# mycophonic/saprobe-alac

Hardware: AMD Instinct MI355X
Metric: Msamples/s decoded (16-bit stereo, 4096-frame packets) (higher is better)
Workload: dtype int32; 1 GPU; 65536 packets/GPU x 16-bit 2-ch 4096-frame ALAC, music-like synthetic, device-resident in/out; packets_per_gpu=65536

## Files before the change

saprobe-alac_amd/csrc/alac_duo.h:

```cpp
#ifndef ALAC_DUO_H
#define ALAC_DUO_H

#include <type_traits>

#include "alac_regular.h"

namespace alac {

constexpr uint32_t DUO_CHUNK = 16;
constexpr int DUO_UN8_MAX = 12;
enum { ROLE_A = 0, ROLE_B = 1, ROLE_BOTH = 2, ROLE_C = 3 };

template <class W, class B, int NA, int OUT, int ROLE, bool F16, bool NARROW, bool EA, bool UN8W = false, bool EC = false, int WMODE = 0>
ALAC_DEV void duo_phase(W& wv, const DevCfg& cfg, const B& bits, RegLane<W>& s, uint32_t size, uint32_t ns,
                        uint32_t n_it, uint32_t hdr_pos, uint32_t den_shift, uint32_t chan_bits, int32_t mix_res,
                        uint32_t mix_sh, uint32_t na_rt, uint32_t shift_pos, uint32_t sb, uint32_t mode) {
    constexpr bool DO_A = ROLE == ROLE_A || ROLE == ROLE_BOTH, DO_B = ROLE == ROLE_B || ROLE == ROLE_BOTH;
    constexpr bool RAW = OUT == OUT_RAW;
    constexpr bool LAST = OUT == OUT_STEREO || OUT == OUT_MONO || RAW;
    constexpr bool CPE = OUT == OUT_STEREO;
    constexpr bool QND = W::kResMem || EC;
    constexpr bool GEN = NA == 0;
    constexpr int NR = GEN ? 1 : NA;
    constexpr bool WRAP = !(NA == 4 || NA == 5 || NA == 6 || NA == 8);
    constexpr uint32_t BIAS = 0x80000000u;
    static_assert(!(EA && EC), "one writer");
    constexpr bool DO_C = (ROLE == ROLE_C || ROLE == ROLE_BOTH) && EC;
    constexpr bool EMIT_A = (EA || EC) && LAST && !RAW;
    constexpr bool DO_EMIT = EMIT_A ? (EC ? DO_C : DO_A) : DO_B;
    constexpr uint32_t CH = EMIT_A ? DUO_CHUNK / 2u : DUO_CHUNK;
    const uint32_t na = GEN ? na_rt : (uint32_t)NA;
    uint32_t kb = cfg.kb;
    ALAC_OWN_REG(kb);
    const uint32_t wb = go_shl(1u, kb) - 1u;
    const uint32_t c31kb = 31u - kb;
    const uint32_t chan_shift = 32u - chan_bits;
    const int32_t den_half = den_shift ? (int32_t)(1u << (den_shift - 1u)) : 0;
    const uint32_t rnd_neg = (1u << den_shift) - 1u;

    int32_t coef[NR];
    uint32_t hb[NR + 1];
    if (DO_B) {
#pragma unroll
        for (int j = 0; j < NR; ++j)
            coef[j] = (!GEN || ((uint32_t)j < na && na != 31)) ? (int32_t)(int16_t)bits.get(hdr_pos + 16u + 16u * (uint32_t)j, 16) : 0;
#pragma unroll
        for (int j = 0; j <= NR; ++j) hb[j] = BIAS;
    }
    uint64_t pk_acc = 0;
    uint32_t pk_n = 0;
    const uint32_t bps = cfg.bps;
    const uint64_t pk_msk = bps == 4 ? 0xffffffffull : ((1ull << (8u * bps)) - 1ull);
    const bool merge_any = DO_EMIT && LAST && !F16 && !RAW && wv.any(sb != 0);
    const bool mode_any = DO_B && wv.any(mode != 0);
    int32_t dprev = 0;
    auto prepass = [&](uint32_t idx, int32_t del) -> int32_t {
        if (!mode_any) return del;
        const int32_t dd = idx == 0 ? del : sext_cs(del + dprev, chan_shift);
        dprev = mode != 0 ? dd : dprev;
        return mode != 0 ? dd : del;
    };
    constexpr bool MID_ONLY = !NARROW && WMODE == 1;
    const bool mid = !NARROW && (MID_ONLY || !wv.any(ns != 0u && chan_bits > 25u));
// ... 66 lines not shown
            const uint32_t pcm = ((uint32_t)l & 0xffffu) | ((uint32_t)r << 16);
            if (FP) wv.st_put(fp_base, jj, pcm, fp_inc);
            else wv.st_push_if(pcm, on);
            return;
        }
        if (cfg.bit_depth == 20) {
            l = (int32_t)((uint32_t)l << 4);
            r = (int32_t)((uint32_t)r << 4);
        }
        if (merge_any) {
            const uint32_t sh_l = sb ? (uint32_t)(sw >> (64u - sb)) : 0u;
            const uint32_t sh_r = (CPE && sb) ? (uint32_t)((sw << sb) >> (64u - sb)) : 0u;
            l = (int32_t)((uint32_t)l << sb) | (int32_t)sh_l;
            r = (int32_t)((uint32_t)r << sb) | (int32_t)sh_r;
        }
        {
            pk_acc |= ((uint64_t)(uint32_t)l & pk_msk) << (8u * pk_n);
            pk_n += on ? bps : 0u;
            bool em = pk_n >= 4u;
            wv.st_push_if((uint32_t)pk_acc, em);
            pk_acc = em ? pk_acc >> 32 : pk_acc;
            pk_n = em ? pk_n - 4u : pk_n;
            if (CPE) {
                pk_acc |= ((uint64_t)(uint32_t)r & pk_msk) << (8u * pk_n);
                pk_n += on ? bps : 0u;
                em = pk_n >= 4u;
                wv.st_push_if((uint32_t)pk_acc, em);
                pk_acc = em ? pk_acc >> 32 : pk_acc;
                pk_n = em ? pk_n - 4u : pk_n;
            }
            pk_acc &= pk_n ? ((1ull << (8u * pk_n)) - 1ull) : 0ull;
        }
    };
    auto put = [&](uint32_t buf, uint32_t j, uint32_t i, int32_t o, int32_t u, uint64_t sw, uint32_t jj, auto fp) {
#pragma unroll
        for (int t = NR; t >= 1; --t) hb[t] = hb[t - 1];
        hb[0] = (uint32_t)o ^ BIAS;
        if (!LAST) *wv.u_row(i) = o;
        else if (EMIT_A) wv.rq_write(buf, CH + j, o);
        else emit(i, o, u, sw, jj, fp);
    };
    constexpr bool PK3 = CPE && LAST && !F16 && !RAW && !EMIT_A;
    constexpr bool PK3C = CPE && LAST && !F16 && !RAW && EMIT_A && EC;
    const bool sb8 = (PK3 || PK3C) && !wv.any(ns != 0u && sb != 8u);
    const bool sb0 = (PK3 || PK3C) && !wv.any(ns != 0u && sb != 0u);
    const bool pk3 = (PK3 || PK3C) && bps == 3u && (sb8 || sb0);
    const uint32_t sh_byte = shift_pos >> 3, sh_bit = shift_pos & 7u;
    auto pk3_block = [&](uint32_t rowq, const int32_t (&vv4)[4], const int32_t (&uu4)[4], uint32_t g0, uint32_t g1, uint32_t g2) {
        const uint32_t w0 = (uint32_t)(((((uint64_t)g0) << 32) | g1) << sh_bit >> 32);
        const uint32_t w1 = (uint32_t)(((((uint64_t)g1) << 32) | g2) << sh_bit >> 32);
        uint32_t lq[4], rq[4];
#pragma unroll
        for (uint32_t j = 0; j < 4u; ++j) {
            const int32_t vv = vv4[j];
            const int32_t mv = NARROW ? ALAC_MUL24(mix_res, vv) : (int32_t)((uint32_t)mix_res * (uint32_t)vv);
            int32_t l = uu4[j] + (int32_t)((uint32_t)vv & nzm) - (mv >> mix_sh);
            int32_t r = (int32_t)((((uint32_t)(l - vv)) & nzm) | ((uint32_t)vv & ~nzm));
            if (sb8) {
                const uint32_t w = j < 2u ? w0 : w1;
                const uint32_t sl = (j & 1u) ? (w >> 8) & 0xffu : w >> 24;
                const uint32_t sr = (j & 1u) ? w & 0xffu : (w >> 16) & 0xffu;
                l = (int32_t)(((uint32_t)l << 8) | sl);
                r = (int32_t)(((uint32_t)r << 8) | sr);
            } else if (cfg.bit_depth == 20) {
                l = (int32_t)((uint32_t)l << 4);
                r = (int32_t)((uint32_t)r << 4);
            }
            lq[j] = (uint32_t)l;
            rq[j] = (uint32_t)r;
        }
        const uint32_t d0 = (lq[0] & 0xffffffu) | (rq[0] << 24);
// ... 47 lines not shown
            const uint32_t i = c * CH + j;
            u_n[j] = 0;
            sw_n[j] = 0;
            if (i < n_it) {
                if (CPE) u_n[j] = *wv.u_row(i);
                if (merge_any && !blocks) sw_n[j] = bits.window_raw(shift_pos + i * sstep_a);
            }
        }
        if (PK3C && blocks && sb8) {
#pragma unroll
            for (uint32_t q = 0; q < CH / 4u; ++q) bits.load12(sh_byte + 2u * (c * CH + 4u * q), g_n[q][0], g_n[q][1], g_n[q][2]);
        }
    };
    auto emit_chunk = [&](uint32_t c) {
        if (PK3C && whole_pk3(c)) {
#pragma unroll
            for (uint32_t q = 0; q < CH / 4u; ++q) {
                int32_t vv4[4], uu4[4];
#pragma unroll
                for (uint32_t j = 0; j < 4u; ++j) {
                    vv4[j] = sq_v[4u * q + j];
                    uu4[j] = u_v[4u * q + j];
                }
                pk3_block(c * CH + 4u * q, vv4, uu4, g_v[q][0], g_v[q][1], g_v[q][2]);
            }
            return;
        }
#pragma unroll
        for (uint32_t j = 0; j < CH; ++j) {
            const uint32_t i = c * CH + j;
            if (i < n_it) emit(i, sq_v[j], u_v[j], sw_v[j], 0u, fp_no{});
        }
        wv.st_step();
    };
    constexpr uint32_t UN = (NARROW && (((F16 || !LAST || RAW || EMIT_A) && NR <= DUO_UN8_MAX) || (UN8W && NR <= 8))) ? 8u : 4u;
    constexpr bool HBM_IN = LAST && !RAW && !EMIT_A;
    constexpr bool RMEM = W::kResMem && ROLE == ROLE_B;
    int32_t dpre[UN];
    uint32_t dpre_row = 0xffffffffu;
    int32_t upre[UN];
    uint64_t spre[UN];
    uint32_t pre_row = 0xffffffffu;
    constexpr uint32_t NSUB = UN / 4u;
    uint32_t gpre[NSUB][3] = {};
    auto prefetch_group = [&](uint32_t row0) {
        pre_row = row0;
#pragma unroll
        for (uint32_t j = 0; j < UN; ++j) {
            upre[j] = 0;
            spre[j] = 0;
            if (CPE) upre[j] = *wv.u_row(row0 + j);
            if (merge_any && !pk3) spre[j] = bits.window_raw(shift_pos + (row0 + j) * sstep_b);
        }
        if (PK3 && pk3 && sb8) {
#pragma unroll
            for (uint32_t q = 0; q < NSUB; ++q) bits.load12(sh_byte + 2u * (row0 + 4u * q), gpre[q][0], gpre[q][1], gpre[q][2]);
        }
    };
    auto predict_chunk = [&](uint32_t c) {
        const uint32_t buf = c & 1u;
        const bool simple = GEN && (na == 0 || na == 31);
        const uint32_t sstep = (CPE ? 2u : 1u) * sb;
        if (!simple && !mode_any && c * CH > na && (c + 1u) * CH <= n_it) {
            auto groups = [&](auto wrap, auto fp) {
                constexpr bool FP = decltype(fp)::value;
#pragma nounroll
// ... 13 lines not shown
                        uv[j] = HBM_IN ? upre[j] : 0;
                        sv[j] = HBM_IN ? spre[j] : 0ull;
                    }
                    uint32_t gq[NSUB][3];
#pragma unroll
                    for (uint32_t q = 0; q < NSUB; ++q) {
                        gq[q][0] = gpre[q][0];
                        gq[q][1] = gpre[q][1];
                        gq[q][2] = gpre[q][2];
                    }
                    if (HBM_IN && row0 + 2u * UN <= steady_end) prefetch_group(row0 + UN);
                    if (RMEM && row0 + 2u * UN <= steady_end) {
                        dpre_row = row0 + UN;
#pragma unroll
                        for (uint32_t j = 0; j < UN; ++j) dpre[j] = wv.rq_read(buf, g + UN + j);
                    }
                    if (PK3 && pk3) {
#pragma unroll
                        for (uint32_t q = 0; q < NSUB; ++q) {
                            int32_t vv4[4], uu4[4];
#pragma unroll
                            for (uint32_t j = 0; j < 4u; ++j) {
                                const int32_t vv = predict_q(dv[4u * q + j], wrap);
#pragma unroll
                                for (int t = NR; t >= 1; --t) hb[t] = hb[t - 1];
                                hb[0] = (uint32_t)vv ^ BIAS;
                                vv4[j] = vv;
                                uu4[j] = uv[4u * q + j];
                            }
                            pk3_block(row0 + 4u * q, vv4, uu4, gq[q][0], gq[q][1], gq[q][2]);
                        }
                        continue;
                    }
#pragma unroll
                    for (uint32_t j = 0; j < UN; ++j)
                        put(buf, g + j, c * CH + g + j, predict_q(dv[j], wrap), uv[j], sv[j], j, fp);
                    if (FP) wv.st_advance(fp_inc);
                    if (LAST && !EMIT_A) wv.st_step();
                }
            };
            auto run_groups = [&](auto wrap) {
                if (FP_OK) {
                    const uint32_t c_end = (c + 1u) * CH;
                    const bool ends_here = ns > c * CH && ns < c_end;
                    if (!wv.any(ends_here)) {
                        fp_inc = ns >= c_end ? UN : 0u;
                        groups(wrap, fp_yes{});
                        return;
                    }
                    groups(wrap, fp_no{});
                    if (ends_here) (void)wv.st_finish();
                    return;
                }
                groups(wrap, fp_no{});
            };
            if (WRAP) {
                constexpr uint32_t T = 32767u - CH;
                uint32_t far = 0;
#pragma unroll
                for (int j = 0; j < NR; ++j) far = umax(far, (uint32_t)coef[j] + T);
                if (!wv.any(far > 2u * T)) {
                    run_groups(wrap_no{});
                    return;
                }
            }
            run_groups(wrap_yes{});
            return;
        }
#pragma nounroll
        for (uint32_t j = 0; j < CH; ++j) {
            const uint32_t i = c * CH + j;
            if (i >= n_it) break;
            const int32_t qv = wv.rq_read(buf, j);
            const int32_t del = prepass(i, QND ? gol_unfold((uint32_t)qv) : qv);
            int32_t o;
            if (i == 0 || (GEN && na == 0)) o = del;
            else if (i <= na || (GEN && na == 31)) o = sext_cs(del + (int32_t)(hb[0] ^ BIAS), chan_shift);
            else o = predict(del, wrap_yes{});
            put(buf, j, i, o, (CPE && !EMIT_A) ? *wv.u_row(i) : 0,
                (!EMIT_A && merge_any) ? bits.window_raw(shift_pos + i * sstep) : 0ull, 0u, fp_no{});
            if (LAST && !EMIT_A) wv.st_step();
            if (FP_OK && i + 1u == ns) (void)wv.st_finish();
        }
    };

    const uint32_t nch = (n_it + CH - 1u) / CH;
    const uint32_t iters = nch + (EMIT_A ? 2u : 1u);
    for (uint32_t c = 0; c < iters; ++c) {
        if (DO_A) {
            if (EMIT_A && !EC && c >= 2u) fetch_chunk(c - 2u);
            if (c < nch) golomb_chunk(c);
        }
        if (DO_B) {
            if (c >= 1u && c <= nch) predict_chunk(c - 1u);
        }
        if (DO_A && EMIT_A && !EC) {
            if (c >= 2u) emit_chunk(c - 2u);
        }
        if (DO_C && EMIT_A) {
            if (c >= 2u) {
#pragma unroll
                for (uint32_t j = 0; j < CH; ++j) {
                    u_v[j] = u_n[j];
                    sw_v[j] = sw_n[j];
                }
#pragma unroll
                for (uint32_t q = 0; q < CH / 4u; ++q) {
                    g_v[q][0] = g_n[q][0];
                    g_v[q][1] = g_n[q][1];
                    g_v[q][2] = g_n[q][2];
                }
            }
            if (c >= 1u && c <= nch) fetch_mem_ahead(c - 1u);
            if (c >= 2u) {
                fetch_chunk(c - 2u);
                emit_chunk(c - 2u);
            }
        }
        wv.duo_sync();
    }
    if (DO_EMIT && LAST) wv.st_tail(pk_acc, pk_n);
    if (!LAST) wv.duo_sync_mem();
}

template <class W, class B, int T, int OUT, int LPP, int NAC = 0>
ALAC_DEV void duo_phase_lanes(W& wv, const B& bits, uint32_t q, uint32_t n_it, uint32_t hdr_pos, uint32_t den_shift,
                              uint32_t chan_bits, uint32_t na_rt) {
    static_assert(LPP == 2 || LPP == 4, "lanes per packet");
    static_assert(LPP == 2 ? NAC == 0 : (NAC >= 1 && (NAC + 3) / 4 == T), "four lanes: T = ceil(order / 4)");
    const uint32_t na = NAC != 0 ? (uint32_t)NAC : na_rt;
    constexpr bool LAST = OUT != OUT_UTILE;
    constexpr uint32_t CH = LAST ? DUO_CHUNK / 2u : DUO_CHUNK;
    constexpr uint32_t BIAS = 0x80000000u;
    const bool wraps = order_wraps16(na);
    const uint32_t chan_shift = 32u - chan_bits;
    const int32_t den_half = den_shift ? (int32_t)(1u << (den_shift - 1u)) : 0;
    const int32_t dh0 = q == 0u ? den_half : 0;
    const uint32_t rnd_neg = (1u << den_shift) - 1u;
    const uint32_t q0m = q == 0u ? 0xffffffffu : 0u;
    const uint32_t up1 = q < 3u ? 0xffffffffu : 0u, up2 = q < 2u ? 0xffffffffu : 0u, up3 = q < 1u ? 0xffffffffu : 0u;
    int32_t coef[T], wneg[T], m[T];
    uint32_t g[T + 1];
#pragma unroll
    for (int t = 0; t < T; ++t) {
        const uint32_t jt = q * (uint32_t)T + (uint32_t)t;
        const bool have = jt < na;
        coef[t] = have ? (int32_t)(int16_t)bits.get(hdr_pos + 16u + 16u * jt, 16) : 0;
        wneg[t] = have ? -(int32_t)(na - jt) : 0;
        m[t] = have ? 1 : 0;
        g[t] = BIAS;
    }
    g[T] = BIAS;
    int32_t prev = 0;
    constexpr int QTOP = NAC != 0 ? (NAC - 1) / T : 1, TTOP = NAC != 0 ? NAC - QTOP * T : T;
    const bool top_last = na == 2u * (uint32_t)T;

    auto step = [&](uint32_t i, uint32_t nd, auto plain_c, auto wrap_c) -> int32_t {
        constexpr bool PLAIN = decltype(plain_c)::value, WR = decltype(wrap_c)::value;
// ... 21 lines not shown
                s = ALAC_MAD24(qv[t], wneg[t], s);
            } else {
                acc = ALAC_MUL24(coef[t], e[t]) + acc;
                s = ALAC_MUL24((int32_t)qv[t], wneg[t]) + s;
            }
        }
        if (LPP == 2) rem += (int32_t)(wv.pair_hi((uint32_t)s) & q0m);
        else rem += (int32_t)((wv.template quad_up<1>((uint32_t)s) & up1) + (wv.template quad_up<2>((uint32_t)s) & up2) +
                              (wv.template quad_up<3>((uint32_t)s) & up3));
#pragma unroll
        for (int t = T - 1; t >= 0; --t) {
            const int32_t go = ALAC_MED3_0(rem, m[t]);
            const int32_t delta = (int32_t)ALAC_XAD(sg[t], sgnm, nsg);
            rem = ALAC_MAD24(qv[t], wneg[t], rem);
            int32_t cj = ALAC_MAD24(delta, go, coef[t]);
            if (WR) cj = (int32_t)(int16_t)cj;
            coef[t] = cj;
        }
        const int32_t at = LPP == 2 ? wv.pair_sum(acc) : wv.quad_sum(acc);
        int32_t o = ALAC_SEXT_BITS(del + (int32_t)(topb ^ BIAS) + (at >> den_shift), chan_bits);
        if (!PLAIN) {
            if (i == 0u) o = del;
            else if (i <= na) o = sext_cs(del + prev, chan_shift);
        }
        const uint32_t g0 = LPP == 2 ? wv.pair_from_below(g[T - 1], (uint32_t)o ^ BIAS, q0m) : wv.quad_from_below(g[T - 1], (uint32_t)o ^ BIAS, q0m);
#pragma unroll
        for (int t = T; t >= 1; --t) g[t] = g[t - 1];
        g[0] = g0;
        prev = o;
        return o;
    };
    using yes = std::integral_constant<bool, true>;
    using no = std::integral_constant<bool, false>;
    auto put = [&](uint32_t buf, uint32_t k, uint32_t i, int32_t o) {
        if (!LAST) *wv.u_row(i) = o;
        else wv.rq_write(buf, CH + k, o);
    };
    auto predict_chunk = [&](uint32_t cc) {
        const uint32_t i0 = cc * CH, buf = cc & 1u;
        const uint32_t nst = umin(CH, n_it - i0);
        if (i0 > na && nst == CH) {
            auto run = [&](auto wrap_c) {
                uint32_t dv[CH];
#pragma unroll
                for (uint32_t k = 0; k < CH; ++k) dv[k] = (uint32_t)wv.rq_read(buf, k);
#pragma unroll
                for (uint32_t k = 0; k < CH; ++k) put(buf, k, i0 + k, step(i0 + k, dv[k], yes{}, wrap_c));
            };
            if (wraps) {
                constexpr uint32_t TW = 32767u - CH;
                uint32_t far = 0;
#pragma unroll
                for (int t = 0; t < T; ++t) far = umax(far, (uint32_t)coef[t] + TW);
                if (wv.any(far > 2u * TW)) {
                    run(yes{});
                    return;
                }
            }
            run(no{});
            return;
        }
#pragma nounroll
        for (uint32_t k = 0; k < nst; ++k) {
            const uint32_t nd = (uint32_t)wv.rq_read(buf, k);
            const int32_t o = wraps ? step(i0 + k, nd, no{}, yes{}) : step(i0 + k, nd, no{}, no{});
            put(buf, k, i0 + k, o);
        }
    };
    const uint32_t nch = (n_it + CH - 1u) / CH;
    const uint32_t iters = nch + (LAST ? 2u : 1u);
    for (uint32_t c = 0; c < iters; ++c) {
        if (c >= 1u && c <= nch) predict_chunk(c - 1u);
        wv.duo_sync();
    }
    if (!LAST) wv.duo_sync_mem();
}

template <class W, int OUT, int LPP, class B>
ALAC_DEV void duo_phase_lanes_na(W& wv, uint32_t na, const B& bits, uint32_t q, uint32_t n_it, uint32_t hdr_pos, uint32_t den_shift,
                                 uint32_t chan_bits) {
    if constexpr (LPP == 4) {
#define ALAC_L4(N) \
    case N: duo_phase_lanes<W, B, (N + 3) / 4, OUT, 4, N>(wv, bits, q, n_it, hdr_pos, den_shift, chan_bits, na); break;
        switch (na) {
            ALAC_L4(3) ALAC_L4(4) ALAC_L4(5) ALAC_L4(6) ALAC_L4(7) ALAC_L4(8) ALAC_L4(9) ALAC_L4(10) ALAC_L4(11) ALAC_L4(12)
            ALAC_L4(13) ALAC_L4(14) ALAC_L4(15)
            default: duo_phase_lanes<W, B, 4, OUT, 4, 16>(wv, bits, q, n_it, hdr_pos, den_shift, chan_bits, na); break;
        }
#undef ALAC_L4
    } else {
        switch ((na + 1u) / 2u) {
            case 0:
            case 1:
            case 2: duo_phase_lanes<W, B, 2, OUT, 2>(wv, bits, q, n_it, hdr_pos, den_shift, chan_bits, na); break;
            case 3: duo_phase_lanes<W, B, 3, OUT, 2>(wv, bits, q, n_it, hdr_pos, den_shift, chan_bits, na); break;
            case 4: duo_phase_lanes<W, B, 4, OUT, 2>(wv, bits, q, n_it, hdr_pos, den_shift, chan_bits, na); break;
            case 5: duo_phase_lanes<W, B, 5, OUT, 2>(wv, bits, q, n_it, hdr_pos, den_shift, chan_bits, na); break;
            case 6: duo_phase_lanes<W, B, 6, OUT, 2>(wv, bits, q, n_it, hdr_pos, den_shift, chan_bits, na); break;
            case 7: duo_phase_lanes<W, B, 7, OUT, 2>(wv, bits, q, n_it, hdr_pos, den_shift, chan_bits, na); break;
            default: duo_phase_lanes<W, B, 8, OUT, 2>(wv, bits, q, n_it, hdr_pos, den_shift, chan_bits, na); break;
        }
    }
}

ALAC_DEV bool duo_lanes_key(uint32_t key, bool cpe, uint32_t lanes_min) {
    const uint32_t nu = (key >> 5) & 31u, nv = key & 31u;
    if ((key & KEY_WIDE) != 0u || nu < 3u || nu > 16u) return false;
    if (!cpe) return nu >= lanes_min;
    if (nv < 3u || nv > 16u) return false;
    return umax(nu, nv) >= lanes_min;
}

ALAC_DEV constexpr bool duo_emit_in_a(uint32_t na, bool cpe) { return !cpe && na >= 5u && na <= 16u; }

template <class W, int OUT, int ROLE, bool F16, bool NARROW = true, bool UN8W = false, bool EC = false, int WMODE = 0, class B>
ALAC_DEV void duo_phase_na(W& wv, uint32_t na, const DevCfg& cfg, const B& bits, RegLane<W>& s, uint32_t size,
                           uint32_t ns, uint32_t n_it, uint32_t hdr_pos, uint32_t den_shift, uint32_t chan_bits,
                           int32_t mix_res, uint32_t mix_sh, uint32_t shift_pos, uint32_t sb, uint32_t mode = 0u) {
#define ALAC_DUO_CASE(N)                                                                                              \
    case N:                                                                                                           \
        duo_phase<W, B, N, OUT, ROLE, F16, NARROW, CAN_EA && duo_emit_in_a(N, OUT == OUT_STEREO), UN8W, EC, WMODE>(wv, cfg, bits, s, size, ns, n_it, hdr_pos, \
                                                                       den_shift, chan_bits, mix_res, mix_sh, na,     \
                                                                       shift_pos, sb, mode);                          \
        break;
    constexpr bool CAN_EA = !EC && NARROW && (OUT == OUT_STEREO || OUT == OUT_MONO);
    if (ROLE == ROLE_A || ROLE == ROLE_C) {
        if constexpr (CAN_EA) {
            if (duo_emit_in_a(na, OUT == OUT_STEREO)) {
                duo_phase<W, B, 0, OUT, ROLE, F16, NARROW, true, false, false>(wv, cfg, bits, s, size, ns, n_it, hdr_pos, den_shift,
                                                                            chan_bits, mix_res, mix_sh, na, shift_pos, sb, mode);
                return;
            }
        }
// ... 2 lines not shown
        return;
    }
    switch (na) {
        ALAC_DUO_CASE(1)
        ALAC_DUO_CASE(2)
        ALAC_DUO_CASE(3)
        ALAC_DUO_CASE(4)
        ALAC_DUO_CASE(5)
        ALAC_DUO_CASE(6)
        ALAC_DUO_CASE(7)
        ALAC_DUO_CASE(8)
        ALAC_DUO_CASE(9)
        ALAC_DUO_CASE(10)
        ALAC_DUO_CASE(11)
        ALAC_DUO_CASE(12)
        ALAC_DUO_CASE(13)
        ALAC_DUO_CASE(14)
        ALAC_DUO_CASE(15)
        ALAC_DUO_CASE(16)
        default:
            duo_phase<W, B, 0, OUT, ROLE, F16, NARROW, false, false, EC, WMODE>(wv, cfg, bits, s, size, ns, n_it, hdr_pos, den_shift, chan_bits,
                                                                             mix_res, mix_sh, na, shift_pos, sb, mode);
            break;
    }
#undef ALAC_DUO_CASE
}

template <class W, int ROLE, int WIDE_SEL = -1, int DEPTH_SEL = 0, bool EC = false, int LANES = 0>
ALAC_DEV int32_t decode_regular_duo(W& wv, const DevCfg& cfg, uint32_t key, bool live, const uint8_t* pkt, uint32_t size,
                                    uint32_t avail, uint8_t* out, uint32_t* frames_out, uint32_t q = 0u, uint32_t ns_other = 0u) {
    constexpr bool DO_A = ROLE == ROLE_A || ROLE == ROLE_BOTH, DO_B = ROLE == ROLE_B || ROLE == ROLE_BOTH;
    constexpr bool DO_C = ROLE == ROLE_C || ROLE == ROLE_BOTH;
    constexpr int WM = DEPTH_SEL == 24 ? 1 : 0;
    const BitsT<false> bits{pkt, size, avail};
    const bool cpe = cfg.num_channels == 2;
    const bool wide = WIDE_SEL < 0 ? (key & KEY_WIDE) != 0 : WIDE_SEL != 0;
    const uint32_t na_u = (key >> 5) & 31u, na_v = key & 31u;

    RegLane<W> s;
    s.rd.init(pkt, size);
    s.err = 0;
    s.near = 0;
    s.max_pos = size * 8u + s.rd.bias;

    uint32_t pos = 23;
    uint32_t ns = 0;
    if (live) {
        ns = cfg.frame_length;
        if (bits.get(19, 4) >> 3) {
            ns = bits.get(pos, 32);
            pos += 32;
        }
    }
    const int32_t mix_bits = (int32_t)bits.get(pos, 8);
    const int32_t mix_res = (int32_t)(int8_t)bits.get(pos + 8, 8);
    const uint32_t mix_sh = (uint32_t)mix_bits > 31u ? 31u : (uint32_t)mix_bits;
    const uint32_t hdr_u = pos + 16u;
    const uint32_t hdr_v = hdr_u + 16u + 16u * na_u;
    const uint32_t hu = bits.get(hdr_u, 16);
    const uint32_t hv = bits.get(hdr_v, 16);
    const uint32_t bs = (bits.get(19, 4) >> 1) & 3u;
    const uint32_t shift_pos = cpe ? hdr_v + 16u + 16u * na_v : hdr_v;
    s.set_upos(shift_pos + bs * 8u * (cpe ? 2u : 1u) * ns);
    const uint32_t chan_bits = cfg.bit_depth - 8u * bs + (cpe ? 1u : 0u);
    const uint32_t sb = (cfg.bit_depth == 24 || cfg.bit_depth == 32) ? bs * 8u : 0u;
    const uint32_t n_it = wv.max_u32(LANES != 0 ? umax(ns, ns_other) : ns);
    if constexpr (LANES != 0) {
        static_assert(ROLE == ROLE_B && EC && WIDE_SEL == 0, "a predictor wave beside an entropy and a writer wave, narrow channels");
        if (cpe) {
            duo_phase_lanes_na<W, OUT_UTILE, LANES>(wv, na_u, bits, q, n_it, hdr_u, (hu >> 8) & 0xfu, chan_bits);
            duo_phase_lanes_na<W, OUT_STEREO, LANES>(wv, na_v, bits, q, n_it, hdr_v, (hv >> 8) & 0xfu, chan_bits);
        } else {
            duo_phase_lanes_na<W, OUT_MONO, LANES>(wv, na_u, bits, q, n_it, hdr_u, (hu >> 8) & 0xfu, chan_bits);
        }
        return 0;
    }
    const bool emit_a = !EC && !wide && duo_emit_in_a(cpe ? na_v : na_u, cpe);
    const bool writer = (EC && !wide) ? DO_C : (emit_a ? DO_A : DO_B);
    if (writer && live) wv.st_begin(out);

    s.mean = cfg.mb;
    s.zmode = 0;
    s.zq = 0xffffffffu;
    s.set_pb((cfg.pb * ((hu >> 5) & 7u)) / 4u);
    if (DO_A) s.rd.start(wv, live ? s.pos : s.rd.bias);
    if constexpr (WIDE_SEL != 1) if (!wide) {
        if (cpe) duo_phase_na<W, OUT_UTILE, ROLE, false, true, false, EC>(wv, na_u, cfg, bits, s, size, ns, n_it, hdr_u, (hu >> 8) & 0xfu, chan_bits, mix_res, mix_sh, shift_pos, 0u);
        else duo_phase_na<W, OUT_MONO, ROLE, false, true, false, EC>(wv, na_u, cfg, bits, s, size, ns, n_it, hdr_u, (hu >> 8) & 0xfu, chan_bits, 0, 0, shift_pos, sb);
    }
    if constexpr (WIDE_SEL != 0) if (wide) {
        if (cpe) duo_phase_na<W, OUT_UTILE, ROLE, false, false, false, false, WM>(wv, na_u, cfg, bits, s, size, ns, n_it, hdr_u, (hu >> 8) & 0xfu, chan_bits, mix_res, mix_sh, shift_pos, 0u);
        else duo_phase_na<W, OUT_MONO, ROLE, false, false, false, false, WM>(wv, na_u, cfg, bits, s, size, ns, n_it, hdr_u, (hu >> 8) & 0xfu, chan_bits, 0, 0, shift_pos, sb);
    }
    uint32_t err_chan = 0;
    if (cpe) {
        const bool u_failed = s.err != 0;
        if (!u_failed && ((s.upos() >> 3) > size + 4u || (s.upos() >> 3) > size)) s.err = ST_MALFORMED;
        const int32_t err_u = s.err;
        s.mean = cfg.mb;
        s.zmode = 0;
        s.zq = 0xffffffffu;
        s.set_pb((cfg.pb * ((hv >> 5) & 7u)) / 4u);
        if (DO_A) s.rd.start(wv, (live && s.err == 0) ? s.pos : s.rd.bias);
        if constexpr (WIDE_SEL != 0) if (wide)
            duo_phase_na<W, OUT_STEREO, ROLE, false, false, false, false, WM>(wv, na_v, cfg, bits, s, size, ns, n_it, hdr_v, (hv >> 8) & 0xfu, chan_bits, mix_res, mix_sh, shift_pos, sb);
        if constexpr (WIDE_SEL != 1) if (!wide) {
            if constexpr (DEPTH_SEL == 0 || DEPTH_SEL == 16) if (cfg.bit_depth == 16)
                duo_phase_na<W, OUT_STEREO, ROLE, true, true, false, EC>(wv, na_v, cfg, bits, s, size, ns, n_it, hdr_v, (hv >> 8) & 0xfu, chan_bits, mix_res, mix_sh, shift_pos, sb);
            if constexpr (DEPTH_SEL != 16) if (cfg.bit_depth != 16)
                duo_phase_na<W, OUT_STEREO, ROLE, false, true, DEPTH_SEL == 24, EC>(wv, na_v, cfg, bits, s, size, ns, n_it, hdr_v, (hv >> 8) & 0xfu, chan_bits, mix_res, mix_sh, shift_pos, sb);
        }
        if (err_u == 0 && s.err != 0) err_chan = 1;
    }
    if (writer && live) (void)wv.st_finish();
    if (!DO_A || !live) return 0;
    if (s.err) {
        *frames_out = 0;
        if (s.err == ST_MALFORMED) return ST_MALFORMED;
        const uint32_t stage = cpe ? (uint32_t)(err_chan == 0 ? ALACGPU_STAGE_ENTROPY_U : ALACGPU_STAGE_ENTROPY_V)
                                   : (uint32_t)ALACGPU_STAGE_ENTROPY;
// ... 9 lines not shown
```

saprobe-alac_amd/csrc/alac_gpu.h:

```cpp
#ifndef ALAC_GPU_H
#define ALAC_GPU_H
#include <hip/hip_runtime.h>

#include <algorithm>
#include <cstdio>
#include <cstdlib>
#include <cstring>

#define ALAC_DEV __device__ __forceinline__
#define ALAC_HD __host__ __device__ __forceinline__
#define ALAC_NOINLINE
#define ALAC_MUL24(a, b) __mul24((int)(a), (int)(b))
__device__ __forceinline__ uint32_t alac_sad(uint32_t a, uint32_t b, uint32_t c) {
    uint32_t r;
    asm("v_sad_u32 %0, %1, %2, %3" : "=v"(r) : "v"(a), "v"(b), "v"(c));
    return r;
}
#define ALAC_SAD(a, b, c) alac_sad((uint32_t)(a), (uint32_t)(b), (uint32_t)(c))

__device__ __forceinline__ int32_t alac_sign_med3(int32_t x) {
    int32_t r;
    asm("v_med3_i32 %0, %1, -1, 1" : "=v"(r) : "v"(x));
    return r;
}
// ... 32 lines not shown
    int32_t r;
    asm("v_mad_i32_i24 %0, %1, %2, %3" : "=v"(r) : "v"(a), "s"(negc), "v"(acc));
    return r;
}
#define ALAC_MSUB24(acc, a, c) alac_msub24((int32_t)(acc), (int32_t)(a), -(int32_t)(c))
#define ALAC_SUBSAT(a, b) __builtin_elementwise_sub_sat((uint32_t)(a), (uint32_t)(b))
__device__ __forceinline__ uint32_t alac_ffbh(uint32_t x) {
    uint32_t r;
    asm("v_ffbh_u32 %0, %1" : "=v"(r) : "v"(x));
    return r;
}
#define ALAC_FFBH(x) alac_ffbh((uint32_t)(x))
__device__ __forceinline__ uint32_t alac_bfe(uint32_t x, uint32_t off, uint32_t width) {
    uint32_t r;
    asm("v_bfe_u32 %0, %1, %2, %3" : "=v"(r) : "v"(x), "v"(off), "v"(width));
    return r;
}
#define ALAC_BFE(x, off, width) alac_bfe((uint32_t)(x), (uint32_t)(off), (uint32_t)(width))
__device__ __forceinline__ int32_t alac_sext_bits(int32_t x, uint32_t bits) {
    int32_t r;
    asm("v_bfe_i32 %0, %1, 0, %2" : "=v"(r) : "v"(x), "v"(bits));
    return r;
}
#define ALAC_SEXT_BITS(x, bits) alac_sext_bits((int32_t)(x), (uint32_t)(bits))
#define ALAC_MULU24(a, b) __umul24((unsigned)(a), (unsigned)(b))
#define ALAC_MULHI(a, b) __umulhi((unsigned)(a), (unsigned)(b))
#define ALAC_ALIGNBIT(hi, lo, sh) __builtin_amdgcn_alignbit((unsigned)(hi), (unsigned)(lo), (unsigned)(sh))
__device__ __forceinline__ int32_t alac_med3_0(int32_t x, int32_t m) {
    int32_t r;
    asm("v_med3_i32 %0, %1, 0, %2" : "=v"(r) : "v"(x), "v"(m));
    return r;
}
#define ALAC_MED3_0(x, m) alac_med3_0((int32_t)(x), (int32_t)(m))
#define ALAC_PICK(dst, src) asm volatile("v_mov_b32 %0, %1" : "+v"(dst) : "v"(src))
#define ALAC_OWN_REG(x) asm volatile("" : "+v"(x))
typedef uint32_t alac_u32x4_a4 __attribute__((ext_vector_type(4), aligned(4)));
#define ALAC_LOAD4(q, a, b, c, d)                                                       \
    do {                                                                                \
        const alac_u32x4_a4 v_ = *reinterpret_cast<const alac_u32x4_a4*>(q);            \
        (a) = v_.x;                                                                     \
        (b) = v_.y;                                                                     \
        (c) = v_.z;                                                                     \
        (d) = v_.w;                                                                     \
    } while (0)
typedef int32_t alac_i32x4 __attribute__((ext_vector_type(4)));
#define ALAC_LOAD4_I32(q, a, b, c, d)                                                  \
    do {                                                                               \
        const alac_i32x4 v_ = *reinterpret_cast<const alac_i32x4*>(q);  \
        (a) = v_.x;                                                                    \
        (b) = v_.y;                                                                    \
        (c) = v_.z;                                                                    \
        (d) = v_.w;                                                                    \
    } while (0)
#define ALAC_STORE4(q, a, b, c, d) (*reinterpret_cast<alac_i32x4*>(q) = alac_i32x4{(a), (b), (c), (d)})
#include "alac_wave.h"
#include "alac_regular.h"
#include "alac_duo.h"
#include "alac_split.h"

#define ALAC_PRIO_B_LONG 3
#define ALAC_PRIO_B_MID 2
#define ALAC_PRIO_B_SHORT 1
#define ALAC_PRIO_A 2
#define ALAC_PRIO_C 3

namespace alack {
// ... 315 lines not shown
```

saprobe-alac_amd/csrc/alac_regular.h:

```cpp
#ifndef ALAC_REGULAR_H
#define ALAC_REGULAR_H

#include "alac_wave.h"

#ifndef ALAC_NOINLINE
#define ALAC_NOINLINE
#endif
#ifndef ALAC_UNLIKELY
#define ALAC_UNLIKELY(x) __builtin_expect(!!(x), 0)
#endif
#ifndef ALAC_HD
#define ALAC_HD ALAC_DEV
#endif
#ifndef ALAC_SAD
#define ALAC_SAD(a, b, c) (((a) > (b) ? (a) - (b) : (b) - (a)) + (c))
#endif
#ifndef ALAC_LOAD4
#define ALAC_LOAD4(q, a, b, c, d) \
    do {                         \
        (a) = (q)[0];            \
        (b) = (q)[1];            \
        (c) = (q)[2];            \
        (d) = (q)[3];            \
    } while (0)
// ... 27 lines not shown
#endif
#ifndef ALAC_XAD
#define ALAC_XAD(a, b, c) ((((uint32_t)(a)) ^ ((uint32_t)(b))) + (uint32_t)(c))
#endif
#ifndef ALAC_MSUB24
#define ALAC_MSUB24(acc, a, c) ((int32_t)(acc) - (int32_t)(a) * (int32_t)(c))
#endif
#ifndef ALAC_OWN_REG
#define ALAC_OWN_REG(x) ((void)0)
#endif
#ifndef ALAC_MULU24
#define ALAC_MULU24(a, b) ((uint32_t)(a) * (uint32_t)(b))
#endif
#ifndef ALAC_FFBH
#define ALAC_FFBH(x) ((uint32_t)(x) ? (uint32_t)__builtin_clz((uint32_t)(x)) : 0xffffffffu)
#endif
#ifndef ALAC_SEXT_BITS
#define ALAC_SEXT_BITS(x, bits) ((int32_t)((uint32_t)(x) << (32u - (bits))) >> (32u - (bits)))
#endif
#ifndef ALAC_MED3_0
#define ALAC_MED3_0(x, m) ((x) <= 0 ? 0 : ((x) < (m) ? (x) : (m)))
#endif
#ifndef ALAC_NOT_ADD
#define ALAC_NOT_ADD(a, c) (~(uint32_t)(a) + (uint32_t)(c))
#endif
#ifndef ALAC_ALIGNBIT
#define ALAC_ALIGNBIT(hi, lo, sh) ((uint32_t)(((((uint64_t)(uint32_t)(hi)) << 32) | (uint32_t)(lo)) >> ((sh) & 31u)))
#endif
#ifndef ALAC_MULHI
#define ALAC_MULHI(a, b) ((uint32_t)(((uint64_t)(uint32_t)(a) * (uint64_t)(uint32_t)(b)) >> 32))
#endif
#ifndef ALAC_BFE
#define ALAC_BFE(x, off, width) ((((uint32_t)(x)) >> ((off) & 31u)) & ((1u << ((width) & 31u)) - 1u))
#endif

namespace alac {

constexpr uint32_t KEY_WIDE = 1024;
constexpr uint32_t KEY_IRREGULAR = 2048;
constexpr uint32_t NUM_KEYS = 2049;

ALAC_DEV bool regular_order(uint32_t na) { return na <= 16 || na == 31; }
ALAC_DEV int32_t imax(int32_t a, int32_t b) { return a > b ? a : b; }

ALAC_HD bool lean_config(const DevCfg& cfg) { return cfg.kb != 0 && cfg.pb <= 73u; }

ALAC_DEV uint32_t classify_regular(const DevCfg& cfg, const uint8_t* pkt, uint32_t size, uint32_t avail) {
    if (cfg.num_channels > 2 || cfg.aligned16 == 0 || !lean_config(cfg) ||
        cfg.frame_length > 65536u || cfg.frame_length <= 32u)
        return KEY_IRREGULAR;
    const Bits bits{pkt, size, avail};
    if (size < 12) return KEY_IRREGULAR;
    const uint32_t tag = bits.get(0, 3);
    const bool cpe = cfg.num_channels == 2;
    if (cpe ? tag != 1 : !(tag == 0 || tag == 3)) return KEY_IRREGULAR;
    if (bits.get(7, 12) != 0) return KEY_IRREGULAR;
    const uint32_t hdr = bits.get(19, 4);
    if (hdr & 1u) return KEY_IRREGULAR;
    const uint32_t bs = (hdr >> 1) & 3u;
    if (bs == 3) return KEY_IRREGULAR;
    const uint32_t chan_bits = cfg.bit_depth - 8u * bs + (cpe ? 1u : 0u);
    if (chan_bits < 1 || chan_bits > 33 || cfg.bit_depth < 8u * bs) return KEY_IRREGULAR;
    const uint32_t wide = chan_bits > 23u ? KEY_WIDE : 0u;
    uint32_t pos = 23;
    uint32_t ns = cfg.frame_length;
    if (hdr >> 3) {
// ... 507 lines not shown
```

Before: 256,500 Msamples/s.

## Pack 16-bit U channel in LDS and unmix stereo with packed 16-bit ops

For 16-bit stereo with a writer wave, the predictor now stores the first (U) channel as pairs of 16-bit values per 32-bit row, halving the intermediate buffer traffic. The writer wave fetches the packed U pairs ahead of time and performs the stereo unmix on two samples at once using v_pk_add/sub_u16 and perm-based packing, emitting interleaved L/R words directly. This reduces LDS reads/writes and ALU work per sample, but adds template variants and relies on 16-bit wraparound being exact for the unmix, so it needs the depth to be compiled per sample width.

```diff
diff --git a/saprobe-alac_amd/csrc/alac_duo.h b/saprobe-alac_amd/csrc/alac_duo.h
--- a/saprobe-alac_amd/csrc/alac_duo.h
+++ b/saprobe-alac_amd/csrc/alac_duo.h
@@ -29,6 +29,8 @@
     constexpr bool EMIT_A = (EA || EC) && LAST && !RAW;
     constexpr bool DO_EMIT = EMIT_A ? (EC ? DO_C : DO_A) : DO_B;
     constexpr uint32_t CH = EMIT_A ? DUO_CHUNK / 2u : DUO_CHUNK;
+    constexpr bool U16_OUT = F16 && EC && OUT == OUT_UTILE;
+    constexpr bool C16 = F16 && EC && CPE && EMIT_A;
     const uint32_t na = GEN ? na_rt : (uint32_t)NA;
     uint32_t kb = cfg.kb;
     ALAC_OWN_REG(kb);
@@ -161,11 +163,16 @@
             pk_acc &= pk_n ? ((1ull << (8u * pk_n)) - 1ull) : 0ull;
         }
     };
+    uint32_t u_even = 0;
     auto put = [&](uint32_t buf, uint32_t j, uint32_t i, int32_t o, int32_t u, uint64_t sw, uint32_t jj, auto fp) {
 #pragma unroll
         for (int t = NR; t >= 1; --t) hb[t] = hb[t - 1];
         hb[0] = (uint32_t)o ^ BIAS;
-        if (!LAST) *wv.u_row(i) = o;
+        if (!LAST && U16_OUT) {
+            if (i & 1u) *wv.u_row(i >> 1) = (int32_t)ALAC_PACK_LO16(u_even, o);
+            else if (i + 1u == n_it) *wv.u_row(i >> 1) = o;
+            else u_even = (uint32_t)o;
+        } else if (!LAST) *wv.u_row(i) = o;
         else if (EMIT_A) wv.rq_write(buf, CH + j, o);
         else emit(i, o, u, sw, jj, fp);
     };
@@ -279,6 +286,63 @@
             if (i < n_it) emit(i, sq_v[j], u_v[j], sw_v[j], 0u, fp_no{});
         }
         wv.st_step();
+    };
+    uint32_t up[CH / 2u] = {};
+    auto fetch_u16 = [&](uint32_t c) {
+        if ((c + 1u) * CH <= n_it) {
+            const int32_t* const ub = wv.u_row(c * (CH / 2u));
+            const ptrdiff_t rs = wv.u_row(1u) - wv.u_row(0u);
+#pragma unroll
+            for (uint32_t k = 0; k < CH / 2u; ++k) up[k] = (uint32_t)ub[(ptrdiff_t)k * rs];
+            return;
+        }
+#pragma unroll
+        for (uint32_t k = 0; k < CH / 2u; ++k) {
+            up[k] = 0;
+            if (c * CH + 2u * k < n_it) up[k] = (uint32_t)*wv.u_row(c * (CH / 2u) + k);
+        }
+    };
+    const bool all_mat = C16 && !wv.any(ns != 0u && mix_res == 0);
+    auto emit_chunk16 = [&](uint32_t c) {
+        const uint32_t buf = c & 1u, c0 = c * CH, c_end = c0 + CH;
+        const bool ends_here = ns > c0 && ns < c_end;
+        if (c_end <= n_it && !wv.any(ends_here)) {
+            const uint32_t inc = ns >= c_end ? CH : 0u;
+            int32_t vq[CH];
+#pragma unroll
+            for (uint32_t j = 0; j < CH; ++j) vq[j] = wv.rq_read(buf, CH + j);
+            const uint32_t base = wv.st_group_base(CH);
+            auto pairs = [&](auto mat) {
+                constexpr bool MAT = decltype(mat)::value;
+#pragma unroll
+                for (uint32_t k = 0; k < CH / 2u; ++k) {
+                    const int32_t v0 = vq[2u * k], v1 = vq[2u * k + 1u];
+                    const uint32_t m = ALAC_PACK_LO16(ALAC_MUL24(mix_res, v0) >> mix_sh, ALAC_MUL24(mix_res, v1) >> mix_sh);
+                    const uint32_t v = ALAC_PACK_LO16(v0, v1);
+                    uint32_t l, r = ALAC_PK_SUB16(up[k], m);
+                    if (MAT) {
+                        l = ALAC_PK_ADD16(r, v);
+                    } else {
+                        l = ALAC_PK_ADD16(r, v & nzm);
+                        r = ALAC_BFI(nzm, r, v);
+                    }
+                    wv.st_put(base, 2u * k, ALAC_PACK_LO16(l, r), inc);
+                    wv.st_put(base, 2u * k + 1u, ALAC_PACK_HI16(l, r), inc);
+                }
+            };
+            if (all_mat) pairs(fp_yes{});
+            else pairs(fp_no{});
+            wv.st_advance(inc);
+            wv.st_step();
+            return;
+        }
+#pragma unroll
+        for (uint32_t j = 0; j < CH; ++j) {
+            const uint32_t i = c0 + j;
+            if (i < n_it) emit(i, wv.rq_read(buf, CH + j), (int32_t)(up[j / 2u] >> (16u * (j & 1u))), 0ull, 0u, fp_no{});
+        }
+        wv.st_step();
+        if (ends_here) (void)wv.st_finish();
     };
     constexpr uint32_t UN = (NARROW && (((F16 || !LAST || RAW || EMIT_A) && NR <= DUO_UN8_MAX) || (UN8W && NR <= 8))) ? 8u : 4u;
     constexpr bool HBM_IN = LAST && !RAW && !EMIT_A;
@@ -358,6 +422,20 @@
                         }
                         continue;
                     }
+                    if (U16_OUT) {
+                        int32_t* const ub = wv.u_row(row0 >> 1);
+                        const ptrdiff_t rs = wv.u_row(1u) - wv.u_row(0u);
+#pragma unroll
+                        for (uint32_t j = 0; j < UN; ++j) {
+                            const int32_t o = predict_q(dv[j], wrap);
+#pragma unroll
+                            for (int t = NR; t >= 1; --t) hb[t] = hb[t - 1];
+                            hb[0] = (uint32_t)o ^ BIAS;
+                            if (j & 1u) ub[(ptrdiff_t)(j >> 1) * rs] = (int32_t)ALAC_PACK_LO16(u_even, o);
+                            else u_even = (uint32_t)o;
+                        }
+                        continue;
+                    }
 #pragma unroll
                     for (uint32_t j = 0; j < UN; ++j)
                         put(buf, g + j, c * CH + g + j, predict_q(dv[j], wrap), uv[j], sv[j], j, fp);
@@ -423,7 +501,10 @@
         if (DO_A && EMIT_A && !EC) {
             if (c >= 2u) emit_chunk(c - 2u);
         }
-        if (DO_C && EMIT_A) {
+        if (DO_C && C16) {
+            if (c >= 2u) emit_chunk16(c - 2u);
+            if (c >= 1u && c <= nch) fetch_u16(c - 1u);
+        } else if (DO_C && EMIT_A) {
             if (c >= 2u) {
 #pragma unroll
                 for (uint32_t j = 0; j < CH; ++j) {
@@ -449,7 +530,7 @@
     if (!LAST) wv.duo_sync_mem();
 }
 
-template <class W, class B, int T, int OUT, int LPP, int NAC = 0>
+template <class W, class B, int T, int OUT, int LPP, int NAC = 0, bool U16 = false>
 ALAC_DEV void duo_phase_lanes(W& wv, const B& bits, uint32_t q, uint32_t n_it, uint32_t hdr_pos, uint32_t den_shift,
                               uint32_t chan_bits, uint32_t na_rt) {
     static_assert(LPP == 2 || LPP == 4, "lanes per packet");
@@ -537,8 +618,13 @@
     };
     using yes = std::integral_constant<bool, true>;
     using no = std::integral_constant<bool, false>;
+    uint32_t u_even = 0;
     auto put = [&](uint32_t buf, uint32_t k, uint32_t i, int32_t o) {
-        if (!LAST) *wv.u_row(i) = o;
+        if (!LAST && U16) {
+            if (i & 1u) *wv.u_row(i >> 1) = (int32_t)ALAC_PACK_LO16(u_even, o);
+            else if (i + 1u == n_it) *wv.u_row(i >> 1) = o;
+            else u_even = (uint32_t)o;
+        } else if (!LAST) *wv.u_row(i) = o;
         else wv.rq_write(buf, CH + k, o);
     };
     auto predict_chunk = [&](uint32_t cc) {
@@ -549,6 +635,17 @@
                 uint32_t dv[CH];
 #pragma unroll
                 for (uint32_t k = 0; k < CH; ++k) dv[k] = (uint32_t)wv.rq_read(buf, k);
+                if (!LAST && U16) {
+                    int32_t* const ub = wv.u_row(i0 >> 1);
+                    const ptrdiff_t rs = wv.u_row(1u) - wv.u_row(0u);
+#pragma unroll
+                    for (uint32_t k = 0; k < CH; ++k) {
+                        const int32_t o = step(i0 + k, dv[k], yes{}, wrap_c);
+                        if (k & 1u) ub[(ptrdiff_t)(k >> 1) * rs] = (int32_t)ALAC_PACK_LO16(u_even, o);
+                        else u_even = (uint32_t)o;
+                    }
+                    return;
+                }
 #pragma unroll
                 for (uint32_t k = 0; k < CH; ++k) put(buf, k, i0 + k, step(i0 + k, dv[k], yes{}, wrap_c));
             };
@@ -581,29 +678,29 @@
     if (!LAST) wv.duo_sync_mem();
 }
 
-template <class W, int OUT, int LPP, class B>
+template <class W, int OUT, int LPP, bool U16 = false, class B>
 ALAC_DEV void duo_phase_lanes_na(W& wv, uint32_t na, const B& bits, uint32_t q, uint32_t n_it, uint32_t hdr_pos, uint32_t den_shift,
                                  uint32_t chan_bits) {
     if constexpr (LPP == 4) {
 #define ALAC_L4(N) \
-    case N: duo_phase_lanes<W, B, (N + 3) / 4, OUT, 4, N>(wv, bits, q, n_it, hdr_pos, den_shift, chan_bits, na); break;
+    case N: duo_phase_lanes<W, B, (N + 3) / 4, OUT, 4, N, U16>(wv, bits, q, n_it, hdr_pos, den_shift, chan_bits, na); break;
         switch (na) {
             ALAC_L4(3) ALAC_L4(4) ALAC_L4(5) ALAC_L4(6) ALAC_L4(7) ALAC_L4(8) ALAC_L4(9) ALAC_L4(10) ALAC_L4(11) ALAC_L4(12)
             ALAC_L4(13) ALAC_L4(14) ALAC_L4(15)
-            default: duo_phase_lanes<W, B, 4, OUT, 4, 16>(wv, bits, q, n_it, hdr_pos, den_shift, chan_bits, na); break;
+            default: duo_phase_lanes<W, B, 4, OUT, 4, 16, U16>(wv, bits, q, n_it, hdr_pos, den_shift, chan_bits, na); break;
         }
 #undef ALAC_L4
     } else {
         switch ((na + 1u) / 2u) {
             case 0:
             case 1:
-            case 2: duo_phase_lanes<W, B, 2, OUT, 2>(wv, bits, q, n_it, hdr_pos, den_shift, chan_bits, na); break;
-            case 3: duo_phase_lanes<W, B, 3, OUT, 2>(wv, bits, q, n_it, hdr_pos, den_shift, chan_bits, na); break;
-            case 4: duo_phase_lanes<W, B, 4, OUT, 2>(wv, bits, q, n_it, hdr_pos, den_shift, chan_bits, na); break;
-            case 5: duo_phase_lanes<W, B, 5, OUT, 2>(wv, bits, q, n_it, hdr_pos, den_shift, chan_bits, na); break;
-            case 6: duo_phase_lanes<W, B, 6, OUT, 2>(wv, bits, q, n_it, hdr_pos, den_shift, chan_bits, na); break;
-            case 7: duo_phase_lanes<W, B, 7, OUT, 2>(wv, bits, q, n_it, hdr_pos, den_shift, chan_bits, na); break;
-            default: duo_phase_lanes<W, B, 8, OUT, 2>(wv, bits, q, n_it, hdr_pos, den_shift, chan_bits, na); break;
+            case 2: duo_phase_lanes<W, B, 2, OUT, 2, 0, U16>(wv, bits, q, n_it, hdr_pos, den_shift, chan_bits, na); break;
+            case 3: duo_phase_lanes<W, B, 3, OUT, 2, 0, U16>(wv, bits, q, n_it, hdr_pos, den_shift, chan_bits, na); break;
+            case 4: duo_phase_lanes<W, B, 4, OUT, 2, 0, U16>(wv, bits, q, n_it, hdr_pos, den_shift, chan_bits, na); break;
+            case 5: duo_phase_lanes<W, B, 5, OUT, 2, 0, U16>(wv, bits, q, n_it, hdr_pos, den_shift, chan_bits, na); break;
+            case 6: duo_phase_lanes<W, B, 6, OUT, 2, 0, U16>(wv, bits, q, n_it, hdr_pos, den_shift, chan_bits, na); break;
+            case 7: duo_phase_lanes<W, B, 7, OUT, 2, 0, U16>(wv, bits, q, n_it, hdr_pos, den_shift, chan_bits, na); break;
+            default: duo_phase_lanes<W, B, 8, OUT, 2, 0, U16>(wv, bits, q, n_it, hdr_pos, den_shift, chan_bits, na); break;
         }
     }
 }
@@ -672,6 +769,8 @@
     constexpr bool DO_A = ROLE == ROLE_A || ROLE == ROLE_BOTH, DO_B = ROLE == ROLE_B || ROLE == ROLE_BOTH;
     constexpr bool DO_C = ROLE == ROLE_C || ROLE == ROLE_BOTH;
     constexpr int WM = DEPTH_SEL == 24 ? 1 : 0;
+    constexpr bool U16 = EC && DEPTH_SEL == 16;
+    static_assert(!EC || DEPTH_SEL != 0, "workgroups with a writer wave are compiled per sample width");
     const BitsT<false> bits{pkt, size, avail};
     const bool cpe = cfg.num_channels == 2;
     const bool wide = WIDE_SEL < 0 ? (key & KEY_WIDE) != 0 : WIDE_SEL != 0;
@@ -708,7 +807,7 @@
     if constexpr (LANES != 0) {
         static_assert(ROLE == ROLE_B && EC && WIDE_SEL == 0, "a predictor wave beside an entropy and a writer wave, narrow channels");
         if (cpe) {
-            duo_phase_lanes_na<W, OUT_UTILE, LANES>(wv, na_u, bits, q, n_it, hdr_u, (hu >> 8) & 0xfu, chan_bits);
+            duo_phase_lanes_na<W, OUT_UTILE, LANES, U16>(wv, na_u, bits, q, n_it, hdr_u, (hu >> 8) & 0xfu, chan_bits);
             duo_phase_lanes_na<W, OUT_STEREO, LANES>(wv, na_v, bits, q, n_it, hdr_v, (hv >> 8) & 0xfu, chan_bits);
         } else {
             duo_phase_lanes_na<W, OUT_MONO, LANES>(wv, na_u, bits, q, n_it, hdr_u, (hu >> 8) & 0xfu, chan_bits);
@@ -725,7 +824,7 @@
     s.set_pb((cfg.pb * ((hu >> 5) & 7u)) / 4u);
     if (DO_A) s.rd.start(wv, live ? s.pos : s.rd.bias);
     if constexpr (WIDE_SEL != 1) if (!wide) {
-        if (cpe) duo_phase_na<W, OUT_UTILE, ROLE, false, true, false, EC>(wv, na_u, cfg, bits, s, size, ns, n_it, hdr_u, (hu >> 8) & 0xfu, chan_bits, mix_res, mix_sh, shift_pos, 0u);
+        if (cpe) duo_phase_na<W, OUT_UTILE, ROLE, U16, true, false, EC>(wv, na_u, cfg, bits, s, size, ns, n_it, hdr_u, (hu >> 8) & 0xfu, chan_bits, mix_res, mix_sh, shift_pos, 0u);
         else duo_phase_na<W, OUT_MONO, ROLE, false, true, false, EC>(wv, na_u, cfg, bits, s, size, ns, n_it, hdr_u, (hu >> 8) & 0xfu, chan_bits, 0, 0, shift_pos, sb);
     }
     if constexpr (WIDE_SEL != 0) if (wide) {
diff --git a/saprobe-alac_amd/csrc/alac_gpu.h b/saprobe-alac_amd/csrc/alac_gpu.h
--- a/saprobe-alac_amd/csrc/alac_gpu.h
+++ b/saprobe-alac_amd/csrc/alac_gpu.h
@@ -88,6 +88,20 @@
     return r;
 }
 #define ALAC_MED3_0(x, m) alac_med3_0((int32_t)(x), (int32_t)(m))
+#define ALAC_PACK_LO16(x, y) __builtin_amdgcn_perm((uint32_t)(y), (uint32_t)(x), 0x05040100u)
+#define ALAC_PACK_HI16(x, y) __builtin_amdgcn_perm((uint32_t)(y), (uint32_t)(x), 0x07060302u)
+__device__ __forceinline__ uint32_t alac_pk_add16(uint32_t a, uint32_t b) {
+    uint32_t r;
+    asm("v_pk_add_u16 %0, %1, %2" : "=v"(r) : "v"(a), "v"(b));
+    return r;
+}
+#define ALAC_PK_ADD16(a, b) alac_pk_add16((uint32_t)(a), (uint32_t)(b))
+__device__ __forceinline__ uint32_t alac_pk_sub16(uint32_t a, uint32_t b) {
+    uint32_t r;
+    asm("v_pk_sub_u16 %0, %1, %2" : "=v"(r) : "v"(a), "v"(b));
+    return r;
+}
+#define ALAC_PK_SUB16(a, b) alac_pk_sub16((uint32_t)(a), (uint32_t)(b))
 #define ALAC_PICK(dst, src) asm volatile("v_mov_b32 %0, %1" : "+v"(dst) : "v"(src))
 #define ALAC_OWN_REG(x) asm volatile("" : "+v"(x))
 typedef uint32_t alac_u32x4_a4 __attribute__((ext_vector_type(4), aligned(4)));
diff --git a/saprobe-alac_amd/csrc/alac_regular.h b/saprobe-alac_amd/csrc/alac_regular.h
--- a/saprobe-alac_amd/csrc/alac_regular.h
+++ b/saprobe-alac_amd/csrc/alac_regular.h
@@ -83,6 +83,20 @@
 #endif
 #ifndef ALAC_BFE
 #define ALAC_BFE(x, off, width) ((((uint32_t)(x)) >> ((off) & 31u)) & ((1u << ((width) & 31u)) - 1u))
+#endif
+#ifndef ALAC_PACK_LO16
+#define ALAC_PACK_LO16(x, y) ((((uint32_t)(x)) & 0xffffu) | (((uint32_t)(y)) << 16))
+#endif
+#ifndef ALAC_PACK_HI16
+#define ALAC_PACK_HI16(x, y) ((((uint32_t)(x)) >> 16) | (((uint32_t)(y)) & 0xffff0000u))
+#endif
+#ifndef ALAC_PK_ADD16
+#define ALAC_PK_ADD16(a, b) \
+    (((((uint32_t)(a)) + ((uint32_t)(b))) & 0xffffu) | (((((uint32_t)(a)) >> 16) + (((uint32_t)(b)) >> 16)) << 16))
+#endif
+#ifndef ALAC_PK_SUB16
+#define ALAC_PK_SUB16(a, b) \
+    (((((uint32_t)(a)) - ((uint32_t)(b))) & 0xffffu) | (((((uint32_t)(a)) >> 16) - (((uint32_t)(b)) >> 16)) << 16))
 #endif
 
 namespace alac {
```

Result: faster. 259,700 Msamples/s (median of 6 runs) (+1.2%).
